# HarryL-Git/ampnet

Hardware: AMD Instinct MI355X
Metric: AMPConv edges/sec (fwd+bwd) (higher is better)
Workload: dtype f32

## Files before the change

### ampnet_amd/csrc/edge_mfma_f16x2.hip

```cpp
#include "edge_wave16.h"

namespace {
using namespace wave16;

constexpr int kLoOff = kPlaneBytes + 64;
constexpr int kTileBytes = kLoOff + kPlaneBytes;
constexpr float kPScale = 16384.f;
constexpr float kPUnscale = 1.f / 16384.f;
constexpr float kSqrtDh = 5.656854249492381f;
constexpr float kMasked = -__builtin_inff();

#define MFMA_F16(a, b, c) \
  __builtin_amdgcn_mfma_f32_16x16x32_f16(__builtin_bit_cast(f16x8, a), __builtin_bit_cast(f16x8, b), (c), 0, 0, 0)

__device__ __forceinline__ f32x4 mfma3(const i32x4 &ah, const i32x4 &al, const i32x4 &bh, const i32x4 &bl, f32x4 c) {
  c = MFMA_F16(al, bh, c);
  c = MFMA_F16(ah, bl, c);
  return MFMA_F16(ah, bh, c);
}

__device__ __forceinline__ float tile_max_norm2(const i32x4 &f0, const i32x4 &f1) {
  const float t = fmaxf(groups_sum(frag_sumsq(f0)), groups_sum(frag_sumsq(f1)));
  return __builtin_bit_cast(float, __builtin_amdgcn_readfirstlane(__builtin_bit_cast(int, row16_max(t))));
}
__device__ __forceinline__ float ds_scale(float own2, float other) {
  return plane_scale(2.f * __builtin_sqrtf(own2) * (kSqrtDh * other));
}

__device__ __forceinline__ void cd_frag2(const f32x4 &t0, float t1_0, i32x4 &hi, i32x4 &lo) {
  int h0, l0, h1, l1, h2, l2;
  split2(t0[0], t0[1], h0, l0);
  split2(t0[2], t0[3], h1, l1);
  split2(t1_0, 0.f, h2, l2);
  hi = i32x4{h0, h1, h2, 0};
  lo = i32x4{l0, l1, l2, 0};
}

struct Args {
  ampconv_view_t Q, K, V, dO, O, dK, dV;
  const int32_t *ptr, *idx;
  const float *bounds;
  float *absmax;
  const int32_t *spos;
  float *stats;
  HubArgs hub;
  int64_t n_units;
  int L, H;
};

template <bool QUARTER, int MC>
__device__ __forceinline__ float store_tile(const ampconv_view_t &v, int64_t node, int h, const f32x4 (&T)[MC][2],
                                            float scale, int L, int lane) {
  const int g = lane >> 4, n = lane & 15;
  float m = 0.f;
#pragma unroll
  for (int nt = 0; nt < 2; ++nt) {
    const int i = nt == 0 ? n : (QUARTER ? 16 + (n >> 2) : 16 + n);
    if (i < L && (nt == 0 || !QUARTER || (n & 3) == 0)) {
#pragma unroll
      for (int mc = 0; mc < MC; ++mc) {
        const float4 o = make_float4(T[mc][nt][0] * scale, T[mc][nt][1] * scale, T[mc][nt][2] * scale,
                                     T[mc][nt][3] * scale);
        const int64_t off = node * v.node_stride + (int64_t)h * v.head_stride + (int64_t)i * v.row_stride + 4 * g + 16 * mc;
        *reinterpret_cast<float4 *>(reinterpret_cast<float *>(v.ptr) + off) = o;
        m = finite_abs_max(m, o);
      }
    }
  }
  return m;
}

struct FmtP {
  using Args = ::Args;
  static constexpr int kPlanes = 2, kElemBytes = 4, kLoOff = ::kLoOff, kTileBytes = ::kTileBytes;
  using Frag = wave16::Frag<2>;
  template <bool HALF> using Geom = PairGeom<HALF ? 4 : 8, HALF ? 3 : 5, HALF ? 4 : 8, 2, ::kLoOff>;
  static constexpr bool kHalfZeroLds = true;
  template <bool HALF> static constexpr int mc_tiles() { return HALF ? 1 : 2; }
  static constexpr bool kShadow = true;
  static constexpr float kMasked = ::kMasked, kPMul = kPScale;

  static __device__ __forceinline__ f32x4 mma(const Frag &a, const Frag &b, f32x4 c) { return mfma3(a.p[0], a.p[1], b.p[0], b.p[1], c); }
  static __device__ __forceinline__ Frag cd_frag(const f32x4 &t0, const f32x4 &t1) {
    Frag f;
    cd_frag2(t0, t1[0], f.p[0], f.p[1]);
    return f;
  }

  struct Scales {
    float uq, ug, sc;
  };
  template <bool HALF> static constexpr float inv_sqrt_dh() { return HALF ? 0.25f : 0.17677669529663687f; }
  template <bool HALF> static __device__ __forceinline__ Scales scales(const Args &a) {
    const float uq = 1.f / plane_scale(uniform_ld(a.bounds)), ug = 1.f / plane_scale(uniform_ld(a.bounds + 1));
    return Scales{uq, ug, (kLog2e * inv_sqrt_dh<HALF>() * uq) * uq};
  }
  static __device__ __forceinline__ int64_t qrow(const Args &, int64_t r) { return r; }
  static __device__ __forceinline__ float fwd_scale(const Scales &k, float mean) { return kPUnscale * k.uq * mean; }
  static __device__ __forceinline__ float ds_mul(const Args &a, int, const Frag (&gB)[2]) {
    return ds_scale(tile_max_norm2(gB[0].p[0], gB[1].p[0]), uniform_ld(a.bounds + 2) * plane_scale(uniform_ld(a.bounds)));
  }
  template <bool HALF> static __device__ __forceinline__ float dq_scale(const Args &, const Scales &k, float ss, bool hubp) {
    return (((1.f / ss) * k.uq) * k.ug) * k.uq * (hubp ? 1.f : inv_sqrt_dh<HALF>());
  }

  template <bool HALF>
  static __device__ __forceinline__ float store(const ampconv_view_t &v, int64_t node, int h, const f32x4 (&T)[HALF ? 1 : 2][2],
                                                float scale, bool, int L, int lane) {
    return store_tile<false, HALF ? 1 : 2>(v, node, h, T, scale, L, lane);
  }
  template <bool HALF>
  static __device__ __forceinline__ void store_zero(const ampconv_view_t &v, int64_t node, int h, int L, int lane) {
    constexpr int MC = HALF ? 1 : 2;
    f32x4 Z[MC][2];
#pragma unroll
    for (int mc = 0; mc < MC; ++mc) Z[mc][0] = Z[mc][1] = f32x4{0.f, 0.f, 0.f, 0.f};
    store_tile<false, MC>(v, node, h, Z, 0.f, L, lane);
  }
  static __device__ __forceinline__ void record_absmax(const Args &a, float m) {
    if (a.absmax) wave_record_absmax(a.absmax, m);
  }
};

template <bool FULL, bool HALF>
__global__ __launch_bounds__(64 * kWavesPerBlock, 4) void fwd_f16x2(Args a) { fwd_body<FmtP, FULL, HALF>(a); }
template <bool FULL, bool STATS, bool HALF>
__global__ __launch_bounds__(64 * kWavesPerBlock, 3) void bwd_dst_f16x2(Args a) { bwd_dst_body<FmtP, FULL, STATS, HALF>(a); }

constexpr int kSrcLds = 4 * kTileBytes + 2 * kLmax * 4 + 32;
template <bool FULL, bool STATS, bool HALF>
__global__ __launch_bounds__(64 * kWavesPerBlock, 3) void bwd_src_f16x2(Args a) {
  using G = FmtP::Geom<HALF>;
  constexpr int MC = HALF ? 1 : 2;
  __shared__ __attribute__((aligned(16))) char lds_all[kWavesPerBlock][kSrcLds];
  for_unit<FmtP, HALF>(a, a.dK, &a.dV, [&](const Unit &u) __attribute__((always_inline)) {
    const int lane = u.lane, h = u.h, beg = u.beg, end = u.end;
    const int L = a.L, n = lane & 15;
    char *Qt = lds_all[u.wave], *Gt = Qt + kTileBytes, *Ko = Gt + kTileBytes, *Vo = Ko + kTileBytes;
    const FmtP::Scales k = FmtP::scales<HALF>(a);
    const float ug = k.ug, sc = k.sc;

    if (!FULL || HALF) lds_zero(Qt, 4 * kTileBytes, lane);
    Pair16<G::NLD> qg;
    pair16_load<FULL, G>(qg, slot_ptr<4>(a.K, u.row, h), (unsigned)a.K.row_stride * 4u, slot_ptr<4>(a.V, u.row, h),
                       (unsigned)a.V.row_stride * 4u, L, lane);
    pair16_to_lds<FULL, G, kTileBytes>(Ko, qg, L, lane);
    __builtin_amdgcn_wave_barrier();
    const float ss = ds_scale(tile_max_norm2(rowfrag(Vo, 0, lane), rowfrag(Vo, 1, lane)), uniform_ld(a.bounds + 3) * plane_scale(uniform_ld(a.bounds + 1)));
    f32x4 dKT[MC][2], dVT[MC][2];
#pragma unroll
    for (int mc = 0; mc < MC; ++mc)
      dKT[mc][0] = dKT[mc][1] = dVT[mc][0] = dVT[mc][1] = f32x4{0.f, 0.f, 0.f, 0.f};

    IdxWindow win;
    const unsigned qrb = (unsigned)a.Q.row_stride * 4u, grb = (unsigned)a.dO.row_stride * 4u;
    float *stl = reinterpret_cast<float *>(Vo + kTileBytes);
    float sv = 0.f;
    auto fetch = [&](int p) {
      const int64_t d = idxwin_get<false>(win, a.idx, nullptr, p, end, lane, nullptr);
      pair16_load<FULL, G>(qg, slot_ptr<4>(a.Q, d, h), qrb, slot_ptr<4>(a.dO, d, h), grb, L, lane);
      if (STATS && lane < kStatsPerUnit) sv = a.stats[((int64_t)p * a.H + h) * kStatsPerUnit + lane];
    };
    if (beg < end) {
      idxwin_load<false>(win, a.idx, nullptr, beg, end, lane);
      fetch(beg);
    }
    const bool v0 = FULL || n < L, v1 = (n & 3) == 0 && 16 + (n >> 2) < L;
    for (int p = beg; p < end; ++p) {
      pair16_to_lds<FULL, G, kTileBytes>(Qt, qg, L, lane);
      if (STATS && lane < kStatsPerUnit) stl[lane] = sv;
      if (p + 1 < end) fetch(p + 1);
      __builtin_amdgcn_wave_barrier();

      f32x4 S[2][2], dP[2][2];
      {
        i32x4 kh[2], kl[2], vh[2], vl[2];
#pragma unroll
        for (int nt = 0; nt < 2; ++nt) {
          kh[nt] = rowfrag(Ko, nt, lane);
          kl[nt] = rowfrag(Ko + kLoOff, nt, lane);
          vh[nt] = rowfrag(Vo, nt, lane);
          vl[nt] = rowfrag(Vo + kLoOff, nt, lane);
        }
#pragma unroll
        for (int mt = 0; mt < 2; ++mt) {
          const i32x4 ah = rowfrag(Qt, mt, lane), al = rowfrag(Qt + kLoOff, mt, lane);
          const i32x4 bh = rowfrag(Gt, mt, lane), bl = rowfrag(Gt + kLoOff, mt, lane);
#pragma unroll
          for (int nt = 0; nt < 2; ++nt) {
            S[mt][nt] = mfma3(ah, al, kh[nt], kl[nt], f32x4{0.f, 0.f, 0.f, 0.f});
            dP[mt][nt] = mfma3(bh, bl, vh[nt], vl[nt], f32x4{0.f, 0.f, 0.f, 0.f});
          }
        }
      }
      if (STATS) {
        const int g = lane >> 4;
        const f32x4 l0 = *reinterpret_cast<const f32x4 *>(stl + 4 * g), d0 = *reinterpret_cast<const f32x4 *>(stl + kLmax + 4 * g);
        const float l1 = stl[16 + g], d1 = stl[kLmax + 16 + g];
#pragma unroll
        for (int mt = 0; mt < 2; ++mt) {
#pragma unroll
          for (int q = 0; q < (mt == 0 ? 4 : 1); ++q) {
            const bool vr = FULL || (mt == 0 ? 4 * g + q : 16 + g) < L;
            const float ls = !vr ? 0.f : mt == 0 ? l0[q] : l1, dl = !vr ? 0.f : mt == 0 ? d0[q] : d1;
            const float s0 = (v0 && vr) ? S[mt][0][q] : kMasked, s1 = (v1 && vr) ? S[mt][1][q] : kMasked;
            const float p0 = fast_exp2(fmaf(s0, sc, -ls)), p1 = fast_exp2(fmaf(s1, sc, -ls));
            S[mt][0][q] = p0 * kPScale;
            S[mt][1][q] = p1 * kPScale;
            dP[mt][0][q] = p0 * (dP[mt][0][q] - dl) * ss;
            dP[mt][1][q] = p1 * (dP[mt][1][q] - dl) * ss;
          }
        }
      } else {
#pragma unroll
      for (int mt = 0; mt < 2; ++mt) {
#pragma unroll
        for (int q = 0; q < (mt == 0 ? 4 : 1); ++q) {
          const float s0 = v0 ? S[mt][0][q] : kMasked, s1 = v1 ? S[mt][1][q] : kMasked;
          const float m = row16_max(fmaxf(s0, s1));
          float p0 = fast_exp2((s0 - m) * sc), p1 = fast_exp2((s1 - m) * sc);
          const float rinv = fast_rcp(row16_sum(p0 + p1));
          p0 *= rinv;
          p1 *= rinv;
          const float delta = row16_sum(fmaf(p0, dP[mt][0][q], p1 * dP[mt][1][q]));
          S[mt][0][q] = p0 * kPScale;
          S[mt][1][q] = p1 * kPScale;
          dP[mt][0][q] = p0 * (dP[mt][0][q] - delta) * ss;
          dP[mt][1][q] = p1 * (dP[mt][1][q] - delta) * ss;
        }
      }
      }
      {
        i32x4 ph[2], pl[2], gh[MC], gl[MC];
        TR_PRE_READ();
#pragma unroll
        for (int mc = 0; mc < MC; ++mc) {
          gh[mc] = colfrag(Gt, mc, lane);
          gl[mc] = colfrag(Gt + kLoOff, mc, lane);
        }
#pragma unroll
        for (int nt = 0; nt < 2; ++nt) cd_frag2(S[0][nt], S[1][nt][0], ph[nt], pl[nt]);
        TR_FRAG_FENCE();
#pragma unroll
        for (int mc = 0; mc < MC; ++mc)
#pragma unroll
          for (int nt = 0; nt < 2; ++nt) dVT[mc][nt] = mfma3(gh[mc], gl[mc], ph[nt], pl[nt], dVT[mc][nt]);
        TR_WAR_GUARD();
      }
      {
        i32x4 sh[2], sl[2], qh[MC], ql[MC];
#pragma unroll
        for (int mc = 0; mc < MC; ++mc) {
          qh[mc] = colfrag(Qt, mc, lane);
          ql[mc] = colfrag(Qt + kLoOff, mc, lane);
        }
#pragma unroll
        for (int nt = 0; nt < 2; ++nt) cd_frag2(dP[0][nt], dP[1][nt][0], sh[nt], sl[nt]);
        TR_FRAG_FENCE();
#pragma unroll
        for (int mc = 0; mc < MC; ++mc)
#pragma unroll
          for (int nt = 0; nt < 2; ++nt) dKT[mc][nt] = mfma3(qh[mc], ql[mc], sh[nt], sl[nt], dKT[mc][nt]);
      }
      __builtin_amdgcn_wave_barrier();
    }
    const bool hubp = a.hub.mode == 2;
    float m = store_tile<true, MC>(a.dK, u.onode, h, dKT, FmtP::dq_scale<HALF>(a, k, ss, hubp), L, lane);
    m = fmaxf(m, store_tile<true, MC>(a.dV, u.onode, h, dVT, kPUnscale * ug, L, lane));
    FmtP::record_absmax(a, m);
  });
}

typedef void (*EdgeKernel)(Args);
int launch_fwd(Args &a, int L, bool half, hipStream_t st) {
  static const EdgeKernel k[2][2] = WAVE16_KERNELS(fwd_f16x2);
  return launch_wave16(k, a, L, half, st);
}
int launch_dst(Args &a, int L, bool half, hipStream_t st) {
  static const EdgeKernel k[2][2][2] = {WAVE16_KERNELS_STATS(bwd_dst_f16x2, false), WAVE16_KERNELS_STATS(bwd_dst_f16x2, true)};
  return launch_wave16(k[a.stats != nullptr], a, L, half, st);
}
int launch_src(Args &a, int L, bool half, hipStream_t st) {
  static const EdgeKernel k[2][2][2] = {WAVE16_KERNELS_STATS(bwd_src_f16x2, false), WAVE16_KERNELS_STATS(bwd_src_f16x2, true)};
  return launch_wave16(k[a.stats != nullptr], a, L, half, st);
}

inline bool plane_view_ok(const ampconv_view_t &v, int dh) {
  return v.ptr && ((uintptr_t)v.ptr % 16 == 0) && v.head_stride == dh && (v.node_stride % 4 == 0) && (v.row_stride % 4 == 0);
}
inline bool f32_view_ok(const ampconv_view_t &v) {
  return v.ptr && ((uintptr_t)v.ptr % 16 == 0) && (v.head_stride % 4 == 0) && (v.node_stride % 4 == 0) && (v.row_stride % 4 == 0);
}
int check_shape(int64_t n, int L, int D, int H, const float *bounds) {
  if (L <= 0 || D <= 0 || H <= 0 || D % H != 0 || n < 0 || !bounds) return AMPCONV_E_BADARG;
  if (L > kLmax || (D / H != DH && D / H != DH / 2)) return AMPCONV_E_DTYPE;
  return AMPCONV_OK;
}

}

extern "C" int ampconv_planes_supported(int L, int D, int H) {
  return L >= 1 && L <= kLmax && H > 0 && D % H == 0 && (D / H == DH || D / H == DH / 2);
}

extern "C" int ampconv_fwd_edge_planes(ampconv_view_t Q, ampconv_view_t K, ampconv_view_t V, const int32_t *rowptr,
                                       const int32_t *col, int64_t n_rows, int L, int D, int H, ampconv_view_t O,
                                       const void *hub_plan, int64_t hub_chunks, void *hub_ws, const float *bounds,
                                       void *stream) {
  if (int rc = check_shape(n_rows, L, D, H, bounds)) return rc;
  if (n_rows == 0) return AMPCONV_OK;
  if (!plane_view_ok(Q, D / H) || !plane_view_ok(K, D / H) || !plane_view_ok(V, D / H) || !f32_view_ok(O) || !rowptr) return AMPCONV_E_BADARG;
  hipStream_t st = (hipStream_t)stream;
  Args a{};
  a.Q = Q; a.K = K; a.V = V;
  a.ptr = rowptr; a.idx = col; a.bounds = bounds; a.L = L; a.H = H;
  auto run = [&](int64_t n, HubArgs hub, const ampconv_view_t *o, float *) {
    a.hub = hub; a.n_units = n * H; a.O = o[0];
    return launch_fwd(a, L, D / H == DH / 2, st);
  };
  return run_edge_pass(run, n_rows, {O}, hub_plan, hub_chunks, hub_ws, L, D, H, rowptr, {1.f}, 0, nullptr, st);
}

extern "C" int ampconv_bwd_edge_dst_planes(ampconv_view_t Q, ampconv_view_t K, ampconv_view_t V, ampconv_view_t dObar,
                                           const int32_t *rowptr, const int32_t *col, int64_t n_rows, int L, int D, int H,
                                           ampconv_view_t dQ, const void *hub_plan, int64_t hub_chunks, void *hub_ws,
                                           const float *bounds, const int32_t *spos, float *stats, float *out_absmax,
                                           void *stream) {
  if (int rc = check_shape(n_rows, L, D, H, bounds)) return rc;
  if (stats && (!spos || (uintptr_t)stats % 16 != 0)) return AMPCONV_E_BADARG;
  if (n_rows == 0) return AMPCONV_OK;
  if (!plane_view_ok(Q, D / H) || !plane_view_ok(K, D / H) || !plane_view_ok(V, D / H) || !plane_view_ok(dObar, D / H) || !f32_view_ok(dQ) || !rowptr)
    return AMPCONV_E_BADARG;
  hipStream_t st = (hipStream_t)stream;
  Args a{};
  a.Q = Q; a.K = K; a.V = V; a.dO = dObar;
  a.ptr = rowptr; a.idx = col; a.bounds = bounds; a.L = L; a.H = H;
  a.spos = spos; a.stats = stats;
  auto run = [&](int64_t n, HubArgs hub, const ampconv_view_t *o, float *absmax) {
    a.hub = hub; a.n_units = n * H; a.O = o[0]; a.absmax = absmax;
    return launch_dst(a, L, D / H == DH / 2, st);
  };
  return run_edge_pass(run, n_rows, {dQ}, hub_plan, hub_chunks, hub_ws, L, D, H, nullptr,
                       {1.f / sqrtf((float)(D / H))}, 0, out_absmax, st);
}

extern "C" int ampconv_bwd_edge_src_planes(ampconv_view_t Q, ampconv_view_t K, ampconv_view_t V, ampconv_view_t dObar,
                                           const int32_t *cscptr, const int32_t *crow, int64_t n_src, int L, int D, int H,
                                           ampconv_view_t dK, ampconv_view_t dV, const void *hub_plan, int64_t hub_chunks,
                                           void *hub_ws, const float *bounds, const float *stats, float *out_absmax,
                                           void *stream) {
  if (int rc = check_shape(n_src, L, D, H, bounds)) return rc;
  if (stats && (uintptr_t)stats % 16 != 0) return AMPCONV_E_BADARG;
  if (n_src == 0) return AMPCONV_OK;
  if (!plane_view_ok(Q, D / H) || !plane_view_ok(K, D / H) || !plane_view_ok(V, D / H) || !plane_view_ok(dObar, D / H) || !f32_view_ok(dK) ||
      !f32_view_ok(dV) || !cscptr)
    return AMPCONV_E_BADARG;
  hipStream_t st = (hipStream_t)stream;
  Args a{};
  a.Q = Q; a.K = K; a.V = V; a.dO = dObar;
  a.ptr = cscptr; a.idx = crow; a.bounds = bounds; a.L = L; a.H = H;
  a.stats = const_cast<float *>(stats);
  auto run = [&](int64_t n, HubArgs hub, const ampconv_view_t *o, float *absmax) {
    a.hub = hub; a.n_units = n * H; a.dK = o[0]; a.dV = o[1]; a.absmax = absmax;
    return launch_src(a, L, D / H == DH / 2, st);
  };
  return run_edge_pass(run, n_src, {dK, dV}, hub_plan, hub_chunks, hub_ws, L, D, H, nullptr,
                       {1.f / sqrtf((float)(D / H)), 1.f}, 0, out_absmax, st);
}
```

### ampnet_amd/csrc/edge_wave16.h

```cpp
#pragma once
#include "plane16.h"

namespace wave16 {
using namespace plane16;

constexpr int kWavesPerBlock = 4;
constexpr int DH = 32;
constexpr int kRowBytes = DH * 2;
constexpr int kPlaneBytes = kLmax * kRowBytes;

template <int P>
struct Frag {
  i32x4 p[P];
};

struct Unit {
  int lane, wave;
  int64_t row, onode;
  int h, beg, end, deg;
};
template <class Fmt, bool HALF, class Body>
__device__ __forceinline__ void for_unit(const typename Fmt::Args &a, const ampconv_view_t &out0, const ampconv_view_t *out1,
                                         const Body &body) {
  Unit u;
  u.lane = threadIdx.x & 63;
  u.wave = __builtin_amdgcn_readfirstlane(threadIdx.x >> 6);
  const int64_t unit = (int64_t)blockIdx.x * kWavesPerBlock + u.wave;
  if (unit >= a.n_units) return;
  if (!map_unit(a.hub, a.ptr, unit, a.n_units, a.H, u.row, u.onode, u.h, u.beg, u.end, u.deg)) return;
  if (u.beg >= u.end && a.hub.mode != 2) {
    Fmt::template store_zero<HALF>(out0, u.onode, u.h, a.L, u.lane);
    if (out1) Fmt::template store_zero<HALF>(*out1, u.onode, u.h, a.L, u.lane);
    return;
  }
  body(u);
}

template <class T>
__device__ __forceinline__ T uniform_ld(const T *p) {
  return *(const __attribute__((address_space(4))) T *)p;
}

template <int EB>
__device__ __forceinline__ const char *slot_ptr(const ampconv_view_t &v, int64_t n, int h) {
  return reinterpret_cast<const char *>(v.ptr) + EB * (n * v.node_stride + (int64_t)h * v.head_stride);
}

template <int LPR_, int NLD_, int CHUNKS_, int PLANES_, int LO_OFF_ = 0>
struct PairGeom {
  static constexpr int LPR = LPR_, RPL = 64 / LPR_, NLD = NLD_, CHUNKS = CHUNKS_, CPP = LPR_ / PLANES_, LO_OFF = LO_OFF_;
};
template <int N>
struct Pair16 {
  i32x4 v[N];
};

template <bool FULL, class G>
__device__ __forceinline__ void pair16_load(Pair16<G::NLD> &t, const char *baseA, unsigned strideA, const char *baseB,
                                          unsigned strideB, int L, int lane) {
  const int r = lane / G::LPR, q = lane % G::LPR;
#pragma unroll
  for (int i = 0; i < G::NLD; ++i) {
    const int R = r + G::RPL * i;
    const bool isB = R >= kLmax;
    const int j = isB ? R - kLmax : R;
    const bool valid = (R < 2 * kLmax) && (FULL || j < L) && (G::CHUNKS == G::LPR || q < G::CHUNKS);
    if (G::CHUNKS < G::LPR) t.v[i] = i32x4{0, 0, 0, 0};
    const unsigned off = (unsigned)j * (isB ? strideB : strideA) + 16u * (unsigned)q;
    const char *p = (isB ? baseB : baseA) + off;
    if (valid) t.v[i] = *reinterpret_cast<const i32x4 *>(p);
  }
}

template <bool FULL, class G, int TILE>
__device__ __forceinline__ void pair16_to_lds(char *tileA, const Pair16<G::NLD> &t, int L, int lane) {
  const int r = lane / G::LPR, q = lane % G::LPR;
#pragma unroll
  for (int i = 0; i < G::NLD; ++i) {
    const int R = r + G::RPL * i;
    const bool isB = R >= kLmax;
    const int j = isB ? R - kLmax : R;
    if ((R < 2 * kLmax) && (FULL || j < L))
      *reinterpret_cast<i32x4 *>(tileA + (isB ? TILE : 0) + (G::CPP < G::LPR && q >= G::CPP ? G::LO_OFF : 0) +
                                 plane_off(j, G::CPP < G::LPR ? q % G::CPP : q)) = t.v[i];
  }
}

__device__ __forceinline__ void lds_zero(char *p, int bytes, int lane) {
  int *z = reinterpret_cast<int *>(p);
  for (int i = lane; i < bytes / 4; i += AMPCONV_WAVE) z[i] = 0;
}

template <int P, bool HALF, bool QUARTER>
__device__ __forceinline__ Frag<P> frag_global(const char *base, unsigned row_bytes, int t, int L, int lane) {
  const int m = lane & 15, kg = lane >> 4;
  const int j = t == 0 ? m : 16 + (QUARTER ? m >> 2 : m);
  Frag<P> f;
#pragma unroll
  for (int pl = 0; pl < P; ++pl) f.p[pl] = i32x4{0, 0, 0, 0};
  if (j < L && (!HALF || kg < 2)) {
#pragma unroll
    for (int pl = P - 1; pl >= 0; --pl)
      f.p[pl] = *reinterpret_cast<const i32x4 *>(base + (unsigned)j * row_bytes + pl * (HALF ? kRowBytes / 2 : kRowBytes) + 16 * kg);
  }
  return f;
}
template <class Fmt>
__device__ __forceinline__ typename Fmt::Frag lds_rowfrag(const char *img, int mt, int lane) {
  typename Fmt::Frag f;
#pragma unroll
  for (int pl = 0; pl < Fmt::kPlanes; ++pl) f.p[pl] = rowfrag(img + pl * Fmt::kLoOff, mt, lane);
  return f;
}
template <class Fmt>
__device__ __forceinline__ typename Fmt::Frag lds_colfrag(const char *img, int mc, int lane) {
  typename Fmt::Frag f;
#pragma unroll
  for (int pl = 0; pl < Fmt::kPlanes; ++pl) f.p[pl] = colfrag(img + pl * Fmt::kLoOff, mc, lane);
  return f;
}

template <bool FULL>
__device__ __forceinline__ float column_softmax(f32x4 &t0, f32x4 &t1, float sc, float mul, float masked, int L, int g) {
  if (!FULL) {
#pragma unroll
    for (int q = 0; q < 4; ++q)
      if (4 * g + q >= L) t0[q] = masked;
    if (16 + g >= L) t1[0] = masked;
  }
  float m = fmaxf(fmaxf(fmaxf(t0[0], t0[1]), fmaxf(t0[2], t0[3])), t1[0]);
  m = groups_max(m);
#pragma unroll
  for (int q = 0; q < 4; ++q) t0[q] = fast_exp2((t0[q] - m) * sc);
  t1[0] = fast_exp2((t1[0] - m) * sc);
  float l = ((t0[0] + t0[1]) + (t0[2] + t0[3])) + t1[0];
  l = groups_sum(l);
  const float inv = fast_rcp(l) * mul;
#pragma unroll
  for (int q = 0; q < 4; ++q) t0[q] *= inv;
  t1[0] *= inv;
  t1[1] = t1[2] = t1[3] = 0.f;
  return fmaf(m, sc, __builtin_amdgcn_logf(l));
}

template <class Fmt, bool FULL, bool HALF>
__device__ __forceinline__ void fwd_body(const typename Fmt::Args &a) {
  using F = typename Fmt::Frag;
  using G = typename Fmt::template Geom<HALF>;
  constexpr int MC = Fmt::template mc_tiles<HALF>(), TB = Fmt::kTileBytes, EB = Fmt::kElemBytes;
  __shared__ __attribute__((aligned(16))) char lds_all[kWavesPerBlock][2 * TB];
  for_unit<Fmt, HALF>(a, a.O, nullptr, [&](const Unit &u) __attribute__((always_inline)) {
    const int lane = u.lane, h = u.h, beg = u.beg, end = u.end;
    const int L = a.L, g = lane >> 4;
    char *Kt = lds_all[u.wave], *Vt = Kt + TB;
    const typename Fmt::Scales k = Fmt::template scales<HALF>(a);

    F qB[2];
    {
      const char *qb = slot_ptr<EB>(a.Q, Fmt::qrow(a, u.row), h);
      const unsigned rb = (unsigned)a.Q.row_stride * EB;
#pragma unroll
      for (int nt = 0; nt < 2; ++nt) qB[nt] = frag_global<Fmt::kPlanes, HALF, false>(qb, rb, nt, L, lane);
    }
    if (!FULL || (HALF && Fmt::kHalfZeroLds)) lds_zero(Kt, 2 * TB, lane);
    f32x4 OT[MC][2];
#pragma unroll
    for (int mc = 0; mc < MC; ++mc) OT[mc][0] = OT[mc][1] = f32x4{0.f, 0.f, 0.f, 0.f};

    Pair16<G::NLD> kv;
    IdxWindow win;
    const unsigned krb = (unsigned)a.K.row_stride * EB, vrb = (unsigned)a.V.row_stride * EB;
    auto fetch = [&](int p) {
      const int64_t s = idxwin_get<false>(win, a.idx, nullptr, p, end, lane, nullptr);
      pair16_load<FULL, G>(kv, slot_ptr<EB>(a.K, s, h), krb, slot_ptr<EB>(a.V, s, h), vrb, L, lane);
    };
    if (beg < end) {
      idxwin_load<false>(win, a.idx, nullptr, beg, end, lane);
      fetch(beg);
    }
    for (int p = beg; p < end; ++p) {
      pair16_to_lds<FULL, G, TB>(Kt, kv, L, lane);
      if (p + 1 < end) fetch(p + 1);
      __builtin_amdgcn_wave_barrier();

      f32x4 S[2][2];
#pragma unroll
      for (int mt = 0; mt < 2; ++mt) {
        const F kA = lds_rowfrag<Fmt>(Kt, mt, lane);
#pragma unroll
        for (int nt = 0; nt < 2; ++nt) S[mt][nt] = Fmt::mma(kA, qB[nt], f32x4{0.f, 0.f, 0.f, 0.f});
      }
      F pB[2];
#pragma unroll
      for (int nt = 0; nt < 2; ++nt) {
        column_softmax<FULL>(S[0][nt], S[1][nt], k.sc, Fmt::kPMul, Fmt::kMasked, L, g);
        if (!Fmt::kShadow) pB[nt] = Fmt::cd_frag(S[0][nt], S[1][nt]);
      }
      F vA[MC];
      if (Fmt::kShadow) TR_PRE_READ();
#pragma unroll
      for (int mc = 0; mc < MC; ++mc) vA[mc] = lds_colfrag<Fmt>(Vt, mc, lane);
      if (Fmt::kShadow) {
#pragma unroll
        for (int nt = 0; nt < 2; ++nt) pB[nt] = Fmt::cd_frag(S[0][nt], S[1][nt]);
      }
      TR_FRAG_FENCE();
#pragma unroll
      for (int mc = 0; mc < MC; ++mc)
#pragma unroll
        for (int nt = 0; nt < 2; ++nt) OT[mc][nt] = Fmt::mma(vA[mc], pB[nt], OT[mc][nt]);
      __builtin_amdgcn_wave_barrier();
    }
    const bool hubp = a.hub.mode == 2;
    Fmt::template store<HALF>(a.O, u.onode, h, OT, Fmt::fwd_scale(k, hubp ? 1.f : (u.deg > 0 ? 1.f / (float)u.deg : 0.f)),
                              hubp, L, lane);
  });
}

template <class Fmt, bool FULL, bool STATS, bool HALF>
__device__ __forceinline__ void bwd_dst_body(const typename Fmt::Args &a) {
  using F = typename Fmt::Frag;
  using G = typename Fmt::template Geom<HALF>;
  constexpr int MC = Fmt::template mc_tiles<HALF>(), TB = Fmt::kTileBytes, EB = Fmt::kElemBytes;
  __shared__ __attribute__((aligned(16))) char lds_all[kWavesPerBlock][2 * TB];
  for_unit<Fmt, HALF>(a, a.O, nullptr, [&](const Unit &u) __attribute__((always_inline)) {
    const int lane = u.lane, h = u.h, beg = u.beg, end = u.end;
    const int L = a.L, g = lane >> 4;
    char *Kt = lds_all[u.wave], *Vt = Kt + TB;
    const typename Fmt::Scales k = Fmt::template scales<HALF>(a);

    F qB[2], gB[2];
    {
      const char *qb = slot_ptr<EB>(a.Q, u.row, h), *gb = slot_ptr<EB>(a.dO, u.row, h);
      const unsigned qrb = (unsigned)a.Q.row_stride * EB, grb = (unsigned)a.dO.row_stride * EB;
#pragma unroll
      for (int nt = 0; nt < 2; ++nt) {
        qB[nt] = frag_global<Fmt::kPlanes, HALF, false>(qb, qrb, nt, L, lane);
        gB[nt] = frag_global<Fmt::kPlanes, HALF, false>(gb, grb, nt, L, lane);
      }
    }
    const float dsm = Fmt::ds_mul(a, u.deg, gB);
    if (!FULL || (HALF && Fmt::kHalfZeroLds)) lds_zero(Kt, 2 * TB, lane);
    f32x4 dQT[MC][2];
#pragma unroll
    for (int mc = 0; mc < MC; ++mc) dQT[mc][0] = dQT[mc][1] = f32x4{0.f, 0.f, 0.f, 0.f};

    Pair16<G::NLD> kv;
    IdxWindow win;
    const unsigned krb = (unsigned)a.K.row_stride * EB, vrb = (unsigned)a.V.row_stride * EB;
    const float *sposf = nullptr;
    if constexpr (STATS) sposf = reinterpret_cast<const float *>(a.spos);
    float cposf = 0.f, cposf_next = 0.f;
    auto fetch = [&](int p) {
      const int64_t s = idxwin_get<STATS>(win, a.idx, sposf, p, end, lane, &cposf_next);
      pair16_load<FULL, G>(kv, slot_ptr<EB>(a.K, s, h), krb, slot_ptr<EB>(a.V, s, h), vrb, L, lane);
    };
    if (beg < end) {
      idxwin_load<STATS>(win, a.idx, sposf, beg, end, lane);
      fetch(beg);
    }
    for (int p = beg; p < end; ++p) {
      pair16_to_lds<FULL, G, TB>(Kt, kv, L, lane);
      cposf = cposf_next;
      if (p + 1 < end) fetch(p + 1);
      __builtin_amdgcn_wave_barrier();

      f32x4 S[2][2], dP[2][2];
      float lse[2], dlt[2];
#pragma unroll
      for (int mt = 0; mt < 2; ++mt) {
        const F kA = lds_rowfrag<Fmt>(Kt, mt, lane);
        const F vA = lds_rowfrag<Fmt>(Vt, mt, lane);
#pragma unroll
        for (int nt = 0; nt < 2; ++nt) {
          S[mt][nt] = Fmt::mma(kA, qB[nt], f32x4{0.f, 0.f, 0.f, 0.f});
          dP[mt][nt] = Fmt::mma(vA, gB[nt], f32x4{0.f, 0.f, 0.f, 0.f});
        }
      }
      F sB[2];
#pragma unroll
      for (int nt = 0; nt < 2; ++nt) {
        lse[nt] = column_softmax<FULL>(S[0][nt], S[1][nt], k.sc, 1.f, Fmt::kMasked, L, g);
        float part = S[1][nt][0] * dP[1][nt][0];
#pragma unroll
        for (int q = 0; q < 4; ++q) part = fmaf(S[0][nt][q], dP[0][nt][q], part);
        const float delta = groups_sum(part);
        dlt[nt] = delta;
#pragma unroll
        for (int q = 0; q < 4; ++q) S[0][nt][q] *= (dP[0][nt][q] - delta) * dsm;
        S[1][nt][0] *= (dP[1][nt][0] - delta) * dsm;
        if (!Fmt::kShadow) sB[nt] = Fmt::cd_frag(S[0][nt], S[1][nt]);
      }
      F kC[MC];
      if (Fmt::kShadow) TR_PRE_READ();
#pragma unroll
      for (int mc = 0; mc < MC; ++mc) kC[mc] = lds_colfrag<Fmt>(Kt, mc, lane);
      if (Fmt::kShadow) {
#pragma unroll
        for (int nt = 0; nt < 2; ++nt) sB[nt] = Fmt::cd_frag(S[0][nt], S[1][nt]);
      }
      TR_FRAG_FENCE();
#pragma unroll
      for (int mc = 0; mc < MC; ++mc)
#pragma unroll
        for (int nt = 0; nt < 2; ++nt) dQT[mc][nt] = Fmt::mma(kC[mc], sB[nt], dQT[mc][nt]);
      if constexpr (STATS) {
        float *st = a.stats + ((int64_t)__builtin_bit_cast(int, cposf) * a.H + h) * kStatsPerUnit;
        if (lane < L) {
          st[lane] = lane < 16 ? lse[0] : lse[1];
          st[kLmax + lane] = lane < 16 ? dlt[0] : dlt[1];
        }
      }
      __builtin_amdgcn_wave_barrier();
    }
    const bool hubp = a.hub.mode == 2;
    const float m = Fmt::template store<HALF>(a.O, u.onode, h, dQT, Fmt::template dq_scale<HALF>(a, k, dsm, hubp), hubp, L, lane);
    Fmt::record_absmax(a, m);
  });
}

#define WAVE16_KERNELS(K) {{K<false, false>, K<true, false>}, {K<false, true>, K<true, true>}}
#define WAVE16_KERNELS_STATS(K, S) {{K<false, S, false>, K<true, S, false>}, {K<false, S, true>, K<true, S, true>}}
template <class Args>
int launch_wave16(void (*const (&kernels)[2][2])(Args), const Args &a, int L, bool half, hipStream_t stream) {
  return launch_wave_units(kernels[half][L == kLmax], a, kWavesPerBlock, stream);
}

}
```

### ampnet_amd/csrc/plane16.h

```cpp
#pragma once
#include "mfma_tile.h"

namespace plane16 {

typedef int i32x4 __attribute__((ext_vector_type(4)));
typedef int i32x2 __attribute__((ext_vector_type(2)));
typedef float f32x2 __attribute__((ext_vector_type(2)));
typedef short s16x4 __attribute__((ext_vector_type(4)));
typedef _Float16 f16x2 __attribute__((ext_vector_type(2)));
typedef _Float16 f16x8 __attribute__((ext_vector_type(8)));
typedef __bf16 bf16x2 __attribute__((ext_vector_type(2)));
typedef __bf16 bf16x8 __attribute__((ext_vector_type(8)));

constexpr float kLog2e = 1.4426950408889634f;

__device__ __forceinline__ int cvt_pk_bf16(float a, float b) {
  f32x2 v = {a, b};
  return __builtin_bit_cast(int, __builtin_convertvector(v, bf16x2));
}
__device__ __forceinline__ int cvt_pk_f16(float a, float b) {
  f32x2 v = {a, b};
  return __builtin_bit_cast(int, __builtin_convertvector(v, f16x2));
}

__device__ __forceinline__ float plane_scale(float bound) {
  int e = (int)((__builtin_bit_cast(unsigned, bound) >> 23) & 0xFFu);
  e = e < 15 ? 15 : (e > 254 ? 254 : e);
  return __builtin_bit_cast(float, (unsigned)(268 - e) << 23);
}
__device__ __forceinline__ float plane_unscale(float bound) { return 1.f / plane_scale(bound); }

__device__ __forceinline__ void split2(float x0, float x1, int &h, int &l) {
  h = cvt_pk_f16(x0, x1);
  const f16x2 hv = __builtin_bit_cast(f16x2, h);
  l = cvt_pk_f16(x0 - (float)hv[0], x1 - (float)hv[1]);
}

__device__ __forceinline__ float frag_sumsq(const i32x4 &f) {
  float s = 0.f;
#pragma unroll
  for (int k = 0; k < 4; ++k) {
    const f16x2 v = __builtin_bit_cast(f16x2, f[k]);
    s = __builtin_amdgcn_fdot2(v, v, s, false);
  }
  return s;
}

__device__ __forceinline__ i32x2 tr_half(const char *p) {
  return __builtin_bit_cast(i32x2, __builtin_amdgcn_ds_read_tr16_b64_v4i16((__attribute__((address_space(3))) s16x4 *)p));
}
__device__ __forceinline__ i32x4 tr_frag(const char *p0, const char *p1) {
  const i32x2 ai = tr_half(p0), bi = tr_half(p1);
  return i32x4{ai[0], ai[1], bi[0], bi[1]};
}

#define TR_FRAG_FENCE()                                    \
  do {                                                     \
    __builtin_amdgcn_sched_barrier(0);                     \
    asm volatile("s_waitcnt lgkmcnt(0)" ::: "memory");     \
    __builtin_amdgcn_sched_barrier(0);                     \
  } while (0)
#define TR_FRAG_FENCE_IDLE()                                                          \
  do {                                                                                \
    __builtin_amdgcn_sched_barrier(0);                                                \
    asm volatile("s_waitcnt lgkmcnt(0)\n\ts_nop 7\n\ts_nop 7" ::: "memory");          \
    __builtin_amdgcn_sched_barrier(0);                                                \
  } while (0)
#define TR_WAR_GUARD()                         \
  do {                                         \
    __builtin_amdgcn_sched_barrier(0);         \
    asm volatile("s_nop 7" ::: "memory");      \
    __builtin_amdgcn_sched_barrier(0);         \
  } while (0)
#define TR_PRE_READ() asm volatile("s_nop 7" ::: "memory")

constexpr int kPlaneRowBytes = 64;
__device__ __forceinline__ int plane_off(int j, int ch) {
  const int f = (4 - (j >> 2)) & 3;
  return j * kPlaneRowBytes + ((ch ^ f) << 4);
}
__device__ __forceinline__ i32x4 rowfrag(const char *img, int mt, int lane) {
  const int m = lane & 15, kg = lane >> 4;
  const int j = mt == 0 ? m : 16 + (m >> 2);
  return *reinterpret_cast<const i32x4 *>(img + plane_off(j, kg));
}
__device__ __forceinline__ i32x4 colfrag(const char *img, int mc, int lane) {
  const int q = (lane >> 2) & 3, pp = lane & 3, kg = lane >> 4;
  const int ch = 2 * mc + (pp >> 1), half = (pp & 1) << 3;
  return tr_frag(img + plane_off(4 * kg + q, ch) + half, img + plane_off(16 + kg, ch) + half);
}

}
```

Measured before the change: 25.96 million.

## Interleave split-f16 MFMA parts across tiles and fold softmax scaling constants

Reorders the three-part hi/lo f16 MFMA emulation so each part is issued across all independent S/dP tiles before the next part. A sched_barrier fence keeps that order, so dependent MFMAs on the same accumulator are spaced apart instead of chained back to back. It also folds the P scale and ds scale constants into precomputed stats and fmaf forms, which removes per-element multiplies. Stats writes are spread over all lanes with a precomputed offset, and log is deferred to the store. The risks are changed rounding order in the accumulation and compiler scheduling constraints that may hurt elsewhere.

```diff
diff --git a/ampnet_amd/csrc/edge_mfma_f16x2.hip b/ampnet_amd/csrc/edge_mfma_f16x2.hip
--- a/ampnet_amd/csrc/edge_mfma_f16x2.hip
+++ b/ampnet_amd/csrc/edge_mfma_f16x2.hip
@@ -7,16 +7,21 @@
 constexpr int kTileBytes = kLoOff + kPlaneBytes;
 constexpr float kPScale = 16384.f;
 constexpr float kPUnscale = 1.f / 16384.f;
+constexpr float kPShift = 14.f;
 constexpr float kSqrtDh = 5.656854249492381f;
 constexpr float kMasked = -__builtin_inff();
 
 #define MFMA_F16(a, b, c) \
   __builtin_amdgcn_mfma_f32_16x16x32_f16(__builtin_bit_cast(f16x8, a), __builtin_bit_cast(f16x8, b), (c), 0, 0, 0)
 
+constexpr int kParts = 3;
+__device__ __forceinline__ f32x4 mfma_part(int part, const i32x4 &ah, const i32x4 &al, const i32x4 &bh, const i32x4 &bl, f32x4 c) {
+  return part == 0 ? MFMA_F16(al, bh, c) : part == 1 ? MFMA_F16(ah, bl, c) : MFMA_F16(ah, bh, c);
+}
 __device__ __forceinline__ f32x4 mfma3(const i32x4 &ah, const i32x4 &al, const i32x4 &bh, const i32x4 &bl, f32x4 c) {
-  c = MFMA_F16(al, bh, c);
-  c = MFMA_F16(ah, bl, c);
-  return MFMA_F16(ah, bh, c);
+#pragma unroll
+  for (int part = 0; part < kParts; ++part) c = mfma_part(part, ah, al, bh, bl, c);
+  return c;
 }
 
 __device__ __forceinline__ float tile_max_norm2(const i32x4 &f0, const i32x4 &f1) {
@@ -81,6 +86,10 @@
   static constexpr float kMasked = ::kMasked, kPMul = kPScale;
 
   static __device__ __forceinline__ f32x4 mma(const Frag &a, const Frag &b, f32x4 c) { return mfma3(a.p[0], a.p[1], b.p[0], b.p[1], c); }
+  static constexpr int kParts = ::kParts;
+  static __device__ __forceinline__ f32x4 mma_part(int part, const Frag &a, const Frag &b, f32x4 c) {
+    return mfma_part(part, a.p[0], a.p[1], b.p[0], b.p[1], c);
+  }
   static __device__ __forceinline__ Frag cd_frag(const f32x4 &t0, const f32x4 &t1) {
     Frag f;
     cd_frag2(t0, t1[0], f.p[0], f.p[1]);
@@ -156,6 +165,8 @@
     const unsigned qrb = (unsigned)a.Q.row_stride * 4u, grb = (unsigned)a.dO.row_stride * 4u;
     float *stl = reinterpret_cast<float *>(Vo + kTileBytes);
     float sv = 0.f;
+    const float ssp = ss * kPUnscale;
+    const float st_mul = lane < kLmax ? 1.f : ssp, st_add = lane < kLmax ? -kPShift : 0.f;
     auto fetch = [&](int p) {
       const int64_t d = idxwin_get<false>(win, a.idx, nullptr, p, end, lane, nullptr);
       pair16_load<FULL, G>(qg, slot_ptr<4>(a.Q, d, h), qrb, slot_ptr<4>(a.dO, d, h), grb, L, lane);
@@ -168,7 +179,7 @@
     const bool v0 = FULL || n < L, v1 = (n & 3) == 0 && 16 + (n >> 2) < L;
     for (int p = beg; p < end; ++p) {
       pair16_to_lds<FULL, G, kTileBytes>(Qt, qg, L, lane);
-      if (STATS && lane < kStatsPerUnit) stl[lane] = sv;
+      if (STATS && lane < kStatsPerUnit) stl[lane] = fmaf(sv, st_mul, st_add);
       if (p + 1 < end) fetch(p + 1);
       __builtin_amdgcn_wave_barrier();
 
@@ -187,9 +198,15 @@
           const i32x4 ah = rowfrag(Qt, mt, lane), al = rowfrag(Qt + kLoOff, mt, lane);
           const i32x4 bh = rowfrag(Gt, mt, lane), bl = rowfrag(Gt + kLoOff, mt, lane);
 #pragma unroll
-          for (int nt = 0; nt < 2; ++nt) {
-            S[mt][nt] = mfma3(ah, al, kh[nt], kl[nt], f32x4{0.f, 0.f, 0.f, 0.f});
-            dP[mt][nt] = mfma3(bh, bl, vh[nt], vl[nt], f32x4{0.f, 0.f, 0.f, 0.f});
+          for (int nt = 0; nt < 2; ++nt) S[mt][nt] = dP[mt][nt] = f32x4{0.f, 0.f, 0.f, 0.f};
+#pragma unroll
+          for (int part = 0; part < kParts; ++part) {
+#pragma unroll
+            for (int nt = 0; nt < 2; ++nt) {
+              S[mt][nt] = mfma_part(part, ah, al, kh[nt], kl[nt], S[mt][nt]);
+              dP[mt][nt] = mfma_part(part, bh, bl, vh[nt], vl[nt], dP[mt][nt]);
+            }
+            MFMA_ORDER_FENCE();
           }
         }
       }
@@ -205,10 +222,10 @@
             const float ls = !vr ? 0.f : mt == 0 ? l0[q] : l1, dl = !vr ? 0.f : mt == 0 ? d0[q] : d1;
             const float s0 = (v0 && vr) ? S[mt][0][q] : kMasked, s1 = (v1 && vr) ? S[mt][1][q] : kMasked;
             const float p0 = fast_exp2(fmaf(s0, sc, -ls)), p1 = fast_exp2(fmaf(s1, sc, -ls));
-            S[mt][0][q] = p0 * kPScale;
-            S[mt][1][q] = p1 * kPScale;
-            dP[mt][0][q] = p0 * (dP[mt][0][q] - dl) * ss;
-            dP[mt][1][q] = p1 * (dP[mt][1][q] - dl) * ss;
+            S[mt][0][q] = p0;
+            S[mt][1][q] = p1;
+            dP[mt][0][q] = p0 * fmaf(dP[mt][0][q], ssp, -dl);
+            dP[mt][1][q] = p1 * fmaf(dP[mt][1][q], ssp, -dl);
           }
         }
       } else {
@@ -219,14 +236,14 @@
           const float s0 = v0 ? S[mt][0][q] : kMasked, s1 = v1 ? S[mt][1][q] : kMasked;
           const float m = row16_max(fmaxf(s0, s1));
           float p0 = fast_exp2((s0 - m) * sc), p1 = fast_exp2((s1 - m) * sc);
-          const float rinv = fast_rcp(row16_sum(p0 + p1));
+          const float rinv = fast_rcp(row16_sum(p0 + p1)) * kPScale;
           p0 *= rinv;
           p1 *= rinv;
-          const float delta = row16_sum(fmaf(p0, dP[mt][0][q], p1 * dP[mt][1][q]));
-          S[mt][0][q] = p0 * kPScale;
-          S[mt][1][q] = p1 * kPScale;
-          dP[mt][0][q] = p0 * (dP[mt][0][q] - delta) * ss;
-          dP[mt][1][q] = p1 * (dP[mt][1][q] - delta) * ss;
+          const float dl = row16_sum(fmaf(p0, dP[mt][0][q], p1 * dP[mt][1][q])) * (ssp * kPUnscale);
+          S[mt][0][q] = p0;
+          S[mt][1][q] = p1;
+          dP[mt][0][q] = p0 * fmaf(dP[mt][0][q], ssp, -dl);
+          dP[mt][1][q] = p1 * fmaf(dP[mt][1][q], ssp, -dl);
         }
       }
       }
diff --git a/ampnet_amd/csrc/edge_wave16.h b/ampnet_amd/csrc/edge_wave16.h
--- a/ampnet_amd/csrc/edge_wave16.h
+++ b/ampnet_amd/csrc/edge_wave16.h
@@ -120,8 +120,12 @@
   return f;
 }
 
+struct ColumnStats {
+  float m, l;
+};
+__device__ __forceinline__ float softmax_lse(const ColumnStats &c, float sc) { return fmaf(c.m, sc, __builtin_amdgcn_logf(c.l)); }
 template <bool FULL>
-__device__ __forceinline__ float column_softmax(f32x4 &t0, f32x4 &t1, float sc, float mul, float masked, int L, int g) {
+__device__ __forceinline__ ColumnStats column_softmax_stats(f32x4 &t0, f32x4 &t1, float sc, float mul, float masked, int L, int g) {
   if (!FULL) {
 #pragma unroll
     for (int q = 0; q < 4; ++q)
@@ -140,7 +144,22 @@
   for (int q = 0; q < 4; ++q) t0[q] *= inv;
   t1[0] *= inv;
   t1[1] = t1[2] = t1[3] = 0.f;
-  return fmaf(m, sc, __builtin_amdgcn_logf(l));
+  return ColumnStats{m, l};
+}
+template <bool FULL>
+__device__ __forceinline__ float column_softmax(f32x4 &t0, f32x4 &t1, float sc, float mul, float masked, int L, int g) {
+  return softmax_lse(column_softmax_stats<FULL>(t0, t1, sc, mul, masked, L, g), sc);
+}
+
+template <class Fmt>
+constexpr int mma_parts() {
+  if constexpr (Fmt::kPlanes > 1) return Fmt::kParts;
+  else return 1;
+}
+template <class Fmt>
+__device__ __forceinline__ f32x4 mma_part(int part, const typename Fmt::Frag &a, const typename Fmt::Frag &b, f32x4 c) {
+  if constexpr (Fmt::kPlanes > 1) return Fmt::mma_part(part, a, b, c);
+  else return Fmt::mma(a, b, c);
 }
 
 template <class Fmt, bool FULL, bool HALF>
@@ -251,6 +270,8 @@
     const float *sposf = nullptr;
     if constexpr (STATS) sposf = reinterpret_cast<const float *>(a.spos);
     float cposf = 0.f, cposf_next = 0.f;
+    const int st_tok = (lane & 15) + (g >= 2 ? 16 : 0), st_off = st_tok + ((g & 1) ? kLmax : 0);
+    const bool st_ok = st_tok < L && (g < 2 || (lane & 15) < 4);
     auto fetch = [&](int p) {
       const int64_t s = idxwin_get<STATS>(win, a.idx, sposf, p, end, lane, &cposf_next);
       pair16_load<FULL, G>(kv, slot_ptr<EB>(a.K, s, h), krb, slot_ptr<EB>(a.V, s, h), vrb, L, lane);
@@ -266,29 +287,43 @@
       __builtin_amdgcn_wave_barrier();
 
       f32x4 S[2][2], dP[2][2];
-      float lse[2], dlt[2];
+      ColumnStats cs[2];
+      float dlt[2];
 #pragma unroll
       for (int mt = 0; mt < 2; ++mt) {
         const F kA = lds_rowfrag<Fmt>(Kt, mt, lane);
         const F vA = lds_rowfrag<Fmt>(Vt, mt, lane);
 #pragma unroll
-        for (int nt = 0; nt < 2; ++nt) {
-          S[mt][nt] = Fmt::mma(kA, qB[nt], f32x4{0.f, 0.f, 0.f, 0.f});
-          dP[mt][nt] = Fmt::mma(vA, gB[nt], f32x4{0.f, 0.f, 0.f, 0.f});
+        for (int nt = 0; nt < 2; ++nt) S[mt][nt] = dP[mt][nt] = f32x4{0.f, 0.f, 0.f, 0.f};
+#pragma unroll
+        for (int part = 0; part < mma_parts<Fmt>(); ++part) {
+#pragma unroll
+          for (int nt = 0; nt < 2; ++nt) {
+            S[mt][nt] = mma_part<Fmt>(part, kA, qB[nt], S[mt][nt]);
+            dP[mt][nt] = mma_part<Fmt>(part, vA, gB[nt], dP[mt][nt]);
+          }
+          if (mma_parts<Fmt>() > 1) MFMA_ORDER_FENCE();
         }
       }
       F sB[2];
 #pragma unroll
       for (int nt = 0; nt < 2; ++nt) {
-        lse[nt] = column_softmax<FULL>(S[0][nt], S[1][nt], k.sc, 1.f, Fmt::kMasked, L, g);
+        cs[nt] = column_softmax_stats<FULL>(S[0][nt], S[1][nt], k.sc, 1.f, Fmt::kMasked, L, g);
         float part = S[1][nt][0] * dP[1][nt][0];
 #pragma unroll
         for (int q = 0; q < 4; ++q) part = fmaf(S[0][nt][q], dP[0][nt][q], part);
         const float delta = groups_sum(part);
         dlt[nt] = delta;
-#pragma unroll
-        for (int q = 0; q < 4; ++q) S[0][nt][q] *= (dP[0][nt][q] - delta) * dsm;
-        S[1][nt][0] *= (dP[1][nt][0] - delta) * dsm;
+        if constexpr (Fmt::kPlanes > 1) {
+          const float dd = delta * dsm;
+#pragma unroll
+          for (int q = 0; q < 4; ++q) S[0][nt][q] *= fmaf(dP[0][nt][q], dsm, -dd);
+          S[1][nt][0] *= fmaf(dP[1][nt][0], dsm, -dd);
+        } else {
+#pragma unroll
+          for (int q = 0; q < 4; ++q) S[0][nt][q] *= (dP[0][nt][q] - delta) * dsm;
+          S[1][nt][0] *= (dP[1][nt][0] - delta) * dsm;
+        }
         if (!Fmt::kShadow) sB[nt] = Fmt::cd_frag(S[0][nt], S[1][nt]);
       }
       F kC[MC];
@@ -306,10 +341,9 @@
         for (int nt = 0; nt < 2; ++nt) dQT[mc][nt] = Fmt::mma(kC[mc], sB[nt], dQT[mc][nt]);
       if constexpr (STATS) {
         float *st = a.stats + ((int64_t)__builtin_bit_cast(int, cposf) * a.H + h) * kStatsPerUnit;
-        if (lane < L) {
-          st[lane] = lane < 16 ? lse[0] : lse[1];
-          st[kLmax + lane] = lane < 16 ? dlt[0] : dlt[1];
-        }
+        const bool t1 = g >= 2;
+        const float lse = softmax_lse(ColumnStats{t1 ? cs[1].m : cs[0].m, t1 ? cs[1].l : cs[0].l}, k.sc), delta = t1 ? dlt[1] : dlt[0];
+        if (st_ok) st[st_off] = (g & 1) ? delta : lse;
       }
       __builtin_amdgcn_wave_barrier();
     }
diff --git a/ampnet_amd/csrc/plane16.h b/ampnet_amd/csrc/plane16.h
--- a/ampnet_amd/csrc/plane16.h
+++ b/ampnet_amd/csrc/plane16.h
@@ -74,6 +74,8 @@
   } while (0)
 #define TR_PRE_READ() asm volatile("s_nop 7" ::: "memory")
 
+#define MFMA_ORDER_FENCE() __builtin_amdgcn_sched_barrier(0x7F6)
+
 constexpr int kPlaneRowBytes = 64;
 __device__ __forceinline__ int plane_off(int j, int ch) {
   const int f = (4 - (j >> 2)) & 3;
```

Result: slower. 25.63 million (-1.3%).
